# sandialabs/implicit-sph

Measured on AMD Instinct MI355X. Metric: pressure-Poisson solves/sec (3D TGV, 1M particles per GPU, GMRES(50)+block-Jacobi ILU(0), tol 1e-8), higher is better.
Workload: dtype f64; 1 GPU; 3D Taylor-Green vortex, 100^3 particles per GPU, Wendland cut=2h (BASELINE configs[1]), state after one Lagrangian step (mode=advect); rows_per_gpu=1000000, global_rows=1000000, nnz_per_gpu=103845090, solver=FGMRES(50) DGKS tol 1e-8, right prec, precond=bjacobi-ilu0, atom_order=lexicographic, library_row_order=bricks, parallelism=domain bricks 1x1x1, RCCL halo + all-reduce, restarts=1, converged=1

## Files before the change

implicit-sph_amd/csrc/block_helmholtz.hpp:

```cpp
#pragma once
#include "assemble.hpp"

namespace isph {

inline bool sell_cols16(isph_ctx *ctx, const Sell &S);


struct BlockHelmholtzArgs {
  HelmholtzArgs h;
  double beta;
  const double *normal;
  int *bcol[9];
  double *bval[9];
};

__global__ __launch_bounds__(kBlock) void k_asm_block_helmholtz(AsmTables T, BlockHelmholtzArgs A,
                                                                const long long *__restrict__ slice_off,
                                                                double *__restrict__ b) {
  const HelmholtzArgs &a = A.h;
  const int i = xcd_block() * blockDim.x + threadIdx.x;
  const int lane = threadIdx.x & 63;
  const int dim = T.dim, d2 = dim * dim;
  if (i >= a.nlocal) {
    const int nslices = (a.nlocal + kSlice - 1) / kSlice;
// ... 335 lines not shown
        }
        if (rc == ISPH_SUCCESS) rc = (T.sorted && n > 32768) ? sell_set_wmax(ctx, B) : sell_sort_rows(ctx, B);
      }
      if (rc == ISPH_SUCCESS && T.sorted && n > 32768 && sell_cols16(ctx, A0->S)) {
        const Sell &S0 = A0->S;
        for (int q = 1; q < d2 && rc == ISPH_SUCCESS; ++q) {
          if (!blk[q]) continue;
          Sell &B = blk[q]->S;
          rc = B.col16.reserve((size_t)S0.stored);
          if (rc == ISPH_SUCCESS) rc = B.wtab.reserve((size_t)S0.nslices * 64);
          if (rc == ISPH_SUCCESS &&
              (hipMemcpyAsync(B.col16.p, S0.col16.p, sizeof(unsigned short) * (size_t)S0.stored, hipMemcpyDeviceToDevice, ctx->stream) != hipSuccess ||
               hipMemcpyAsync(B.wtab.p, S0.wtab.p, sizeof(int) * (size_t)S0.nslices * 64, hipMemcpyDeviceToDevice, ctx->stream) != hipSuccess))
            rc = fail("copy failed", __FILE__, __LINE__);
          if (rc == ISPH_SUCCESS) B.c16_state = 1;
        }
      }
      if (rc == ISPH_SUCCESS && !on_device &&
          hipMemcpyAsync(b_out, db, sizeof(double) * (size_t)lda * dim, hipMemcpyDeviceToHost, ctx->stream) != hipSuccess)
        rc = fail("copy failed", __FILE__, __LINE__);
      if (hipStreamSynchronize(ctx->stream) != hipSuccess || hipGetLastError() != hipSuccess)
        rc = fail("block assembly kernel failed", __FILE__, __LINE__);
    }
    if (rc == ISPH_SUCCESS) {
      long long tot = 0;
      rc = sell_sum_rowlen(ctx, A0->S, &tot);
      for (int q = 0; q < d2; ++q)
        if (blk[q]) blk[q]->S.nnz = tot;
    }
  }
// ... 14 lines not shown
```

implicit-sph_amd/csrc/core.hpp:

```cpp
#pragma once
#include "common.hpp"
#include "order.hpp"
#include "sell.hpp"

namespace isph { struct HostStager; }

struct isph_neigh_layout {
  const void *nptr = nullptr;
  const int *nidx = nullptr, *colmap = nullptr;
  const void *order = nullptr;
  int n = -1, is_sorted = 0;
  isph::DevBuf<long long> off;
  isph::DevBuf<int> idx, len, sorted;
  void release() { off.release(); idx.release(); len.release(); sorted.release(); nptr = nullptr; nidx = colmap = nullptr; order = nullptr; n = -1; is_sorted = 0; }
};

struct isph_neigh_map {
  const int *rowsrc = nullptr, *idmap = nullptr, *colmap_key = nullptr;
  const int *colkey = nullptr;
  const void *order = nullptr;
};

struct isph_table_cache {
  int ntypes = -1, kernel = -1, dim = -1;
// ... 29 lines not shown
  size_t ev_used = 0;
  std::vector<hipEvent_t> hev;
  size_t hev_used = 0;
  hipEvent_t ev0 = nullptr, ev1 = nullptr;
  hipEvent_t ev_fetch = nullptr;
  std::vector<hipEvent_t> ev_ls;
  hipStream_t comm_stream = nullptr;
  hipEvent_t ev_pack = nullptr, ev_halo = nullptr;
  isph::DevBuf<double> xghost;
  isph::HostStager *stager = nullptr;
  bool neigh_hold = false;
  bool pattern_hold = false;
  isph_neigh_layout neigh_cache[2];
  isph_table_cache tables;
  int ordering = 1;
  isph::OrderBox box;
  isph_neigh_map nmap;
  isph::RowOrderPtr held_order;
  const void *held_key[2] = {nullptr, nullptr};
};

namespace isph {
enum ProfClass { PROF_SPMV = 0, PROF_PREC_APPLY, PROF_MULTI_DOT, PROF_MULTI_AXPY_DOT, PROF_MULTI_AXPY_NORM, PROF_ILU_EXTRACT,
                 PROF_ILU_SCHEDULE, PROF_ILU_FACTOR, PROF_NCLASS };
struct ProfScope {
  isph_ctx *c;
  size_t slot = (size_t)-1;
  ProfScope(isph_ctx *ctx, int cls, hipStream_t st = nullptr) : c(ctx) {
    if (!c || !c->profile || (st && st != c->stream)) return;
    if (c->ev_used + 2 > c->ev.size()) {
// ... 60 lines not shown
```

implicit-sph_amd/csrc/ingress.hpp:

```cpp
#pragma once
#include <atomic>
#include <chrono>
#include <cstdint>
#include <condition_variable>
#include <functional>
#include <thread>
#if defined(__x86_64__)
#include <immintrin.h>
#endif

#include "core.hpp"
#include "ilu.hpp"
#include "pattern.hpp"

namespace isph {

#if defined(__x86_64__)
__attribute__((target("avx2"))) inline void stage_copy_avx2(void *dst, const void *src, size_t bytes) {
  char *d = static_cast<char *>(dst);
  const char *s = static_cast<const char *>(src);
  size_t k = 0;
  while (k < bytes && (reinterpret_cast<uintptr_t>(d + k) & 31)) { d[k] = s[k]; ++k; }
  for (; k + 128 <= bytes; k += 128) {
    const __m256i a = _mm256_loadu_si256(reinterpret_cast<const __m256i *>(s + k));
// ... 434 lines not shown
  H->stats[2] = since();
  if (!copies_ok ||
      hipMemcpyAsync(flags, H->flag.p, 2 * sizeof(int), hipMemcpyDeviceToHost, ctx->stream) != hipSuccess ||
      hipStreamSynchronize(ctx->stream) != hipSuccess || hip_err.load())
    if (rc == ISPH_SUCCESS) rc = fail("CSR->SELL conversion failed", __FILE__, __LINE__);
  H->stats[3] = since();
  ISPH_CHECK(rc);
  ISPH_REQUIRE(!bad_col.load(), "column index out of range");
  if (flags[0]) {
    ISPH_CHECK(sell_sort_rows(ctx, S));
    ISPH_CHECK_HIP(hipStreamSynchronize(ctx->stream));
  }
  if (was_unsorted) *was_unsorted = flags[0] != 0;
  if (S.col16.p != nullptr) {
    S.c16_state = flags[1] ? -1 : flags[0] ? 0 : 1;
    if (S.c16_state != 1) { S.col16.release(); S.wtab.release(); }
  }
  ISPH_CHECK_HIP(hipGetLastError());
  if (ctx->pattern_hold && pattern_mappable(S)) {
    DevTmp<int> debase;
    if (gat) {
      std::vector<int> eb((size_t)nrow);
      for (int r = 0; r < nrow; ++r) eb[(size_t)r] = gat->src_rowptr[gat->perm[r]];
      ISPH_CHECK(debase.reserve((size_t)nrow));
      ISPH_CHECK_HIP(hipMemcpyAsync(debase.p, eb.data(), sizeof(int) * (size_t)nrow, hipMemcpyHostToDevice, ctx->stream));
      ISPH_CHECK_HIP(hipStreamSynchronize(ctx->stream));
    }
    ISPH_CHECK(pattern_build<int>(ctx, g.A, g.drp.p, nullptr, ck, gat ? gat->colren : nullptr, gat ? gat->nren : 0,
                                  gat ? debase.p : nullptr));
  }
  H->bytes_sent = sent + 4 * ((long long)nrow + 1);
// ... 232 lines not shown
```

implicit-sph_amd/csrc/isph_capi.hip:

```cpp
#include <algorithm>
#include <numeric>

#include "assemble.hpp"
#include "operators.hpp"
#include "block_helmholtz.hpp"
#include "core.hpp"
#include "ilu.hpp"
#include "krylov.hpp"
#include "sell.hpp"
#include "solver.hpp"
#include "chebyshev.hpp"
#include "amg.hpp"
#include "schwarz.hpp"
#include "gcrodr.hpp"
#include "ingress.hpp"

namespace isph {
thread_local std::string g_last_error;

}

struct isph_overlap {
  int n = 0, next = 0, combine = 0;
  isph_schwarz *inner = nullptr;
// ... 930 lines not shown
    ISPH_CHECK_HIP(hipStreamSynchronize(ctx->stream));
  }
  return ISPH_SUCCESS;
}

int isph_mat_info(const isph_mat *A, long long info[6]) {
  ISPH_REQUIRE(A && info, "NULL argument");
  info[0] = A->S.nrow; info[1] = A->S.ncol; info[2] = A->S.nnz; info[3] = A->S.nslices;
  info[4] = A->S.stored; info[5] = A->S.stored * 12 + ((long long)A->S.nslices + 1) * 8;
  return ISPH_SUCCESS;
}

int isph_mat_column_bits(isph_ctx *ctx, const isph_mat *A, int *bits) {
  ISPH_REQUIRE(ctx && A && bits, "NULL argument");
  *bits = (!A->local && !A->aux && sell_cols16(ctx, A->S)) ? 16 : 32;
  return ISPH_SUCCESS;
}

int isph_mat_export_rows(isph_ctx *ctx, const isph_mat *A, int row_begin, int nrows, long long *rowptr, int *colidx,
                         double *val, long long capacity) {
  ISPH_REQUIRE(ctx && A && rowptr && colidx && val, "NULL argument");
  const Sell &S = A->S;
  ISPH_REQUIRE(row_begin >= 0 && nrows >= 0 && (long long)row_begin + nrows <= S.nrow, "row range outside the matrix");
  if (A->order && nrows > 0) {
    std::vector<int> hperm((size_t)S.nrow), hiperm((size_t)S.nrow);
    ISPH_CHECK_HIP(hipMemcpyAsync(hperm.data(), A->order->perm.p, sizeof(int) * hperm.size(), hipMemcpyDeviceToHost, ctx->stream));
    ISPH_CHECK_HIP(hipMemcpyAsync(hiperm.data(), A->order->iperm.p, sizeof(int) * hiperm.size(), hipMemcpyDeviceToHost, ctx->stream));
    ISPH_CHECK_HIP(hipStreamSynchronize(ctx->stream));
    isph_mat plain;
    plain.S = S;
// ... 142 lines not shown
    return ISPH_SUCCESS;
  }
  ISPH_CHECK(ctx->xdev.reserve((size_t)S.ncol));
  ISPH_CHECK(ctx->bdev.reserve((size_t)(S.nrow > 0 ? S.nrow : 1)));
  ISPH_CHECK_HIP(hipMemcpyAsync(ctx->xdev.p, x, sizeof(double) * nx, hipMemcpyHostToDevice, ctx->stream));
  if (S.ncol > S.nrow && A->halo.npeers == 0) {
    int nbp = 0;
    const int grid = spmv_grid(S.nslices, &nbp);
    hipLaunchKernelGGL((k_sell_spmv<8, false, true>), dim3(grid), dim3(kBlock), 0, ctx->stream, S.nrow, S.nslices, nbp,
                       S.slice_off.p, S.col.p, S.val.p, (const double *)ctx->xdev.p, ctx->bdev.p, (const double *)nullptr,
                       (double *)nullptr);
  } else {
    ISPH_CHECK(spmv_dev(ctx, A, ctx->xdev.p, ctx->bdev.p, nullptr));
  }
  ISPH_CHECK_HIP(hipMemcpyAsync(y, ctx->bdev.p, sizeof(double) * (size_t)S.nrow, hipMemcpyDeviceToHost, ctx->stream));
  ISPH_CHECK_HIP(hipStreamSynchronize(ctx->stream));
  ISPH_CHECK_HIP(hipGetLastError());
  return ISPH_SUCCESS;
}

int isph_spmv_time(isph_ctx *ctx, const isph_mat *A, const double *x_dev, double *y_dev, int reps, int variant, double *avg_ms) {
  ISPH_REQUIRE(ctx && A && x_dev && y_dev && avg_ms && reps > 0, "bad argument");
  const Sell &S = A->S;
  ISPH_REQUIRE(S.ncol == S.nrow || A->halo.npeers > 0, "ghost columns without halo plan");
  if (S.ncol != S.nrow) {
    ISPH_CHECK_HIP(hipEventRecord(ctx->ev0, ctx->stream));
    for (int r = 0; r < reps; ++r) ISPH_CHECK(spmv_dev(ctx, A, x_dev, y_dev, nullptr));
    ISPH_CHECK_HIP(hipEventRecord(ctx->ev1, ctx->stream));
    ISPH_CHECK_HIP(hipEventSynchronize(ctx->ev1));
    float msh = 0.f;
// ... 988 lines not shown
```

implicit-sph_amd/csrc/sell.hpp:

```cpp
#pragma once
#include "common.hpp"

namespace isph {

struct Sell {
  int nrow = 0, ncol = 0, nslices = 0, wmax = 0;
  long long nnz = 0, stored = 0;
  DevBuf<long long> slice_off;
  DevBuf<int> rowlen;
  DevBuf<int> col;
  DevBuf<double> val;
  mutable DevBuf<unsigned short> col16;
  mutable DevBuf<int> wtab;
  mutable int c16_state = 0;
  void release() { slice_off.release(); rowlen.release(); col.release(); val.release(); col16.release(); wtab.release(); c16_state = 0; }
};

__device__ __forceinline__ unsigned amg_like_hash(int x) {
  unsigned h = (unsigned)x;
  h ^= h >> 16; h *= 0x7feb352dU; h ^= h >> 15; h *= 0x846ca68bU; h ^= h >> 16;
  return h;
}

__device__ __forceinline__ long long sell_pos(long long off, int lane, int k) {
  return off + (long long)(k >> 1) * 128 + lane * 2 + (k & 1);
}

template <class OFF>
__global__ void k_csr_rowlen_slicew(int nrow, const OFF *__restrict__ rowptr, int *__restrict__ rowlen,
                                    long long *__restrict__ slice_cnt) {
// ... 496 lines not shown
    const unsigned lo = cc & 0xffffu, hi = cc >> 16;
    acc0 = fma((double)vv.x, x_at<GHOST>(x, xg, nrow, tw[lo >> 10] | (int)(lo & 1023u)), acc0);
    acc1 = fma((double)vv.y, x_at<GHOST>(x, xg, nrow, tw[hi >> 10] | (int)(hi & 1023u)), acc1);
  }
  const int row = slice * kSlice + lane;
  double r = acc0 + acc1;
  if (alpha != 1.0) r *= alpha;
  if (badd != nullptr && row < nrow) r += (double)badd[row];
  if (row < nrow) y[row] = (YT)r;
  if (DOT) {
    const double d = wave_sum(row < nrow ? r * nvec[row] : 0.0);
    if (lane == 0) dot_partial[slice] = d;
  }
}

struct SpmmVecs {
  const double *x[4];
  double *y[4];
};
template <int NV>
__global__ __launch_bounds__(kBlock) void k_sell_spmm16(int nrow, int nslices, int nblocks_padded,
                                                        const long long *__restrict__ slice_off,
                                                        const unsigned short *__restrict__ c16,
                                                        const int *__restrict__ wtab, const double *__restrict__ sval,
                                                        SpmmVecs V) {
  constexpr int UNROLL = 4;
  __shared__ int tab[kBlock / kWave][64];
  const int b = xcd_remap(blockIdx.x, nblocks_padded);
  const int wave = threadIdx.x >> 6;
  const int slice = b * (kBlock / kWave) + wave;
// ... 91 lines not shown
```

implicit-sph_amd/csrc/solver.hpp:

```cpp
#pragma once
#include <cmath>
#include <type_traits>

#include "comm.hpp"
#include "core.hpp"
#include "gmres_host.hpp"
#include "krylov.hpp"

namespace isph {

int prec_apply_dev(isph_ctx *ctx, const isph_prec *M, const double *r, double *z);
int prec_apply_multi_dev(isph_ctx *ctx, const isph_prec *M, int K, const double *const *rs, double *const *zs);

inline int allreduce_inplace(isph_ctx *ctx, double *d, int count) {
  return comm_allreduce(ctx, d, count,  0, ctx->stream);
}

enum { SC_DOT = 0 , SC_Y = 64 , SC_MISC = 128, SC_COUNT = 160 };

constexpr int kMaxLockstep = 4;

inline int ensure_scalars(isph_ctx *ctx) {
  ISPH_CHECK(ctx->dscal.reserve(SC_COUNT * kMaxLockstep));
  ISPH_CHECK(ctx->partial.reserve((size_t)kMaxRedBlocks * 66));
// ... 55 lines not shown
  if (flag.reserve(1) != ISPH_SUCCESS || S.col16.reserve((size_t)S.stored) != ISPH_SUCCESS ||
      S.wtab.reserve((size_t)S.nslices * 64) != ISPH_SUCCESS) { flag.release(); return false; }
  int h = 0;
  if (hipMemsetAsync(flag.p, 0, sizeof(int), ctx->stream) == hipSuccess) {
    hipLaunchKernelGGL(k_sell_compress_cols, dim3((S.nslices + 3) / 4), dim3(kBlock), 0, ctx->stream, 0, S.nslices,
                       (const long long *)S.slice_off.p, (const int *)S.col.p, S.col16.p, S.wtab.p, flag.p);
    if (hipMemcpyAsync(&h, flag.p, sizeof(int), hipMemcpyDeviceToHost, ctx->stream) == hipSuccess &&
        hipStreamSynchronize(ctx->stream) == hipSuccess && hipGetLastError() == hipSuccess && h == 0)
      S.c16_state = 1;
  }
  flag.release();
  if (S.c16_state < 0) { S.col16.release(); S.wtab.release(); }
  return S.c16_state > 0;
}

template <bool DOT, bool LIST, bool GHOST>
inline void spmv_launch(isph_ctx *ctx, const Sell &S, bool c16, int nsl, const int *list, const double *x, const double *xg,
                        double *y, const double *nvec, const double *badd = nullptr, double alpha = 1.0,
                        const float *val32 = nullptr) {
  if (nsl <= 0) return;
  int nbp = 0;
  const int grid = spmv_grid(nsl, &nbp);
  double *part = DOT ? ctx->partial.p : nullptr;
  if (val32 && c16)
    hipLaunchKernelGGL((k_sell_spmv16<8, false, LIST, GHOST, float>), dim3(grid), dim3(kBlock), 0, ctx->stream, S.nrow, nsl, nbp,
                       S.slice_off.p, S.col16.p, S.wtab.p, val32, x, y, nvec, part, list, xg, badd, alpha);
  else if (val32)
    hipLaunchKernelGGL((k_sell_spmv<8, false, true, LIST, GHOST, float>), dim3(grid), dim3(kBlock), 0, ctx->stream, S.nrow, nsl, nbp,
                       S.slice_off.p, S.col.p, val32, x, y, nvec, part, list, xg, badd, alpha);
  else if (c16)
    hipLaunchKernelGGL((k_sell_spmv16<8, DOT, LIST, GHOST>), dim3(grid), dim3(kBlock), 0, ctx->stream, S.nrow, nsl, nbp,
                       S.slice_off.p, S.col16.p, S.wtab.p, S.val.p, x, y, nvec, part, list, xg, badd, alpha);
  else
    hipLaunchKernelGGL((k_sell_spmv<8, DOT, true, LIST, GHOST>), dim3(grid), dim3(kBlock), 0, ctx->stream, S.nrow, nsl, nbp,
                       S.slice_off.p, S.col.p, S.val.p, x, y, nvec, part, list, xg, badd, alpha);
}

inline int spmv_dev(isph_ctx *ctx, const isph_mat *A, const double *x, double *y, const double *nvec, const double *badd = nullptr,
                    double alpha = 1.0, const float *val32 = nullptr) {
  const Sell &S = A->S;
  const bool halo = !A->local && (S.ncol != S.nrow || A->halo.nsend > 0);
  const bool c16 = !A->local && !A->aux && sell_cols16(ctx, S);
  ISPH_REQUIRE(nvec == nullptr || (badd == nullptr && alpha == 1.0 && val32 == nullptr), "spmv: the dot epilogue takes the plain product");
  ProfScope prof((A->local || A->aux) ? nullptr : ctx, PROF_SPMV);
  if (nvec)
    ISPH_CHECK(ctx->partial.reserve((size_t)S.nslices > (size_t)kMaxRedBlocks * 66 ? (size_t)S.nslices : (size_t)kMaxRedBlocks * 66));
  if (!halo) {
    if (nvec) spmv_launch<true, false, false>(ctx, S, c16, S.nslices, nullptr, x, nullptr, y, nvec);
    else spmv_launch<false, false, false>(ctx, S, c16, S.nslices, nullptr, x, nullptr, y, nvec, badd, alpha, val32);
  } else {
    const isph_halo &H = A->halo;
    hipEvent_t *hev = nullptr;
    if (ctx->profile && !A->aux && !A->local) {
      if (ctx->hev_used + 3 > ctx->hev.size())
        for (int k = 0; k < 3; ++k) { hipEvent_t e = nullptr; ISPH_CHECK_HIP(hipEventCreate(&e)); ctx->hev.push_back(e); }
      hev = ctx->hev.data() + ctx->hev_used;
      ctx->hev_used += 3;
    }
    ISPH_CHECK(halo_begin(ctx, A, x, hev));
    if (nvec) spmv_launch<true, true, false>(ctx, S, c16, H.n_int, H.list_int.p, x, nullptr, y, nvec);
    else spmv_launch<false, true, false>(ctx, S, c16, H.n_int, H.list_int.p, x, nullptr, y, nvec, badd, alpha, val32);
    if (hev) ISPH_CHECK_HIP(hipEventRecord(hev[2], ctx->stream));
    ISPH_CHECK_HIP(hipStreamWaitEvent(ctx->stream, ctx->ev_halo, 0));
    if (nvec) spmv_launch<true, true, true>(ctx, S, c16, H.n_bnd, H.list_bnd.p, x, ctx->xghost.p, y, nvec);
// ... 595 lines not shown
```

implicit-sph_amd/hip.py:

```python
import ctypes as C
import sys
import os

import numpy as np

from . import build as _build

UID_BYTES = 128
NOT_SINGULAR, NULLSPACE, PINZERO, DOUBLEDIAG = 0, 1, 2, 3
KERNELS = {"wendland": 0, "quintic": 1, "cubic": 2}

EXPORTS = [
    "isph_ctx_create", "isph_comm_unique_id", "isph_ctx_create_dist", "isph_ctx_create_hostcomm", "isph_ctx_sync", "isph_ctx_destroy", "isph_pool_trim", "isph_pool_set_cap", "isph_set_exact_stream_threshold", "isph_pool_cached_bytes", "isph_pool_info", "isph_halo_create", "isph_halo_forward", "isph_halo_destroy", "isph_prec_create_overlap",
    "isph_last_error", "isph_mat_create_csr", "isph_mat_create_csr_bjacobi", "isph_mat_create_csr_blocks", "isph_mat_create_csr_coords", "isph_mat_create_csr_coords_bjacobi", "isph_ingress_info", "isph_mat_set_halo", "isph_mat_info", "isph_mat_export_csr", "isph_mat_export_rows", "isph_mat_column_bits",
    "isph_mat_destroy", "isph_spmv", "isph_spmv_time", "isph_prec_create", "isph_prec_create_blocks", "isph_prec_create_blocks_fill", "isph_prec_apply",
    "isph_prec_export_ilu", "isph_prec_nnz", "isph_prec_info", "isph_prec_destroy", "isph_solver_params_default", "isph_solve",
    "isph_ctx_set_profile", "isph_ctx_hold_neighbours", "isph_ctx_profile_read", "isph_ctx_set_ordering", "isph_ctx_set_periodic_box", "isph_mat_ordering_info", "isph_mat_ordering", "isph_mat_ordering_faces", "isph_ctx_halo_profile_read", "isph_ctx_comm_info", "isph_device_identity", "isph_assemble_poisson", "isph_assemble_helmholtz", "isph_assemble_solute_transport", "isph_assemble_applied_potential", "isph_compute_volumes", "isph_compute_pnd", "isph_compute_corrections", "isph_gradient", "isph_divergence", "isph_correct_velocity_pressure",
    "isph_advance_begin", "isph_advance_end", "isph_compute_shift", "isph_apply_shift", "isph_shift_particles",
    "isph_solve_block", "isph_assemble_block_helmholtz", "isph_amg_params_default", "isph_prec_create_amg", "isph_prec_amg_levels", "isph_prec_amg_info",
    "isph_prec_amg_export", "isph_prec_amg_aggregates", "isph_prec_amg_path",
    "isph_schwarz_params_default", "isph_prec_create_schwarz", "isph_prec_schwarz_info", "isph_prec_schwarz_timing", "isph_prec_schwarz_export",
    "isph_pb_params_default", "isph_assemble_poisson_boltzmann", "isph_pb_residual", "isph_pb_jacobian", "isph_solve_poisson_boltzmann",
    "isph_compute_normals", "isph_csf_params_default", "isph_csf_phase_normal", "isph_csf_force", "isph_surface_tension_csf", "isph_pairwise_force",
    "isph_smooth_field", "isph_ek_params_default", "isph_electrostatic_force", "isph_random_stress_tensor", "isph_random_stress_force",
    "isph_force_from_random_stress", "isph_cheb_params_default", "isph_prec_create_chebyshev", "isph_prec_value_bits", "isph_prec_cycle_bits",
    "isph_prec_eig_estimate",
    "isph_ilu_params_default", "isph_prec_create_ilu",
    "isph_nlist_build", "isph_nlist_info", "isph_nlist_get", "isph_nlist_destroy",
    "isph_ctx_hold_pattern", "isph_mat_update_values", "isph_mat_pattern_info", "isph_prec_refactor",
# ... 125 lines not shown
                                          C.c_int, C.c_void_p]
        L.isph_mat_create_csr_bjacobi.argtypes = [C.c_void_p, C.c_int, C.c_int, C.c_void_p, C.c_void_p, C.c_void_p,
                                                  C.c_int, C.c_void_p, C.c_void_p]
        L.isph_mat_create_csr_blocks.argtypes = [C.c_void_p, C.c_int, C.c_int, C.c_void_p, C.c_void_p, C.c_void_p,
                                                 C.c_int, C.c_void_p, C.c_void_p, C.c_void_p]
        L.isph_mat_create_csr_coords.argtypes = [C.c_void_p, C.c_int, C.c_int, C.c_void_p, C.c_void_p, C.c_void_p, C.c_int,
                                                 C.c_void_p, C.c_void_p, C.c_void_p, C.c_void_p]
        L.isph_mat_create_csr_coords_bjacobi.argtypes = [C.c_void_p, C.c_int, C.c_int, C.c_void_p, C.c_void_p, C.c_void_p, C.c_int,
                                                         C.c_void_p, C.c_void_p, C.c_void_p, C.c_void_p, C.c_void_p]
        L.isph_mat_set_halo.argtypes = [C.c_void_p, C.c_void_p, C.c_int, C.c_void_p, C.c_void_p, C.c_void_p,
                                        C.c_void_p]
        L.isph_mat_info.argtypes = [C.c_void_p, C.c_void_p]
        L.isph_mat_export_csr.argtypes = [C.c_void_p, C.c_void_p, C.c_void_p, C.c_void_p, C.c_void_p]
        L.isph_mat_export_rows.argtypes = [C.c_void_p, C.c_void_p, C.c_int, C.c_int, C.c_void_p, C.c_void_p, C.c_void_p, C.c_longlong]
        L.isph_mat_column_bits.argtypes = [C.c_void_p, C.c_void_p, C.c_void_p]
        L.isph_mat_destroy.argtypes = [C.c_void_p]
        L.isph_spmv.argtypes = [C.c_void_p, C.c_void_p, C.c_void_p, C.c_void_p, C.c_int]
        L.isph_spmv_time.argtypes = [C.c_void_p, C.c_void_p, C.c_void_p, C.c_void_p, C.c_int, C.c_int, C.c_void_p]
        L.isph_prec_create.argtypes = [C.c_void_p, C.c_void_p, C.c_char_p, C.c_int, C.c_void_p]
        L.isph_prec_create_blocks.argtypes = [C.c_void_p, C.c_void_p, C.c_int, C.c_void_p, C.c_void_p]
        L.isph_prec_create_blocks_fill.argtypes = [C.c_void_p, C.c_void_p, C.c_int, C.c_void_p, C.c_int, C.c_void_p]
        L.isph_prec_apply.argtypes = [C.c_void_p, C.c_void_p, C.c_void_p, C.c_void_p, C.c_int]
        L.isph_prec_export_ilu.argtypes = [C.c_void_p, C.c_void_p, C.c_void_p, C.c_void_p, C.c_void_p]
        L.isph_prec_destroy.argtypes = [C.c_void_p]
        L.isph_prec_info.argtypes = [C.c_void_p, C.c_void_p, C.c_void_p]
        L.isph_solve.argtypes = [C.c_void_p, C.c_void_p, C.c_void_p, C.c_void_p, C.c_void_p, C.c_int, C.c_int,
                                 C.c_int, C.c_void_p, C.c_void_p, C.c_void_p, C.c_int]
        L.isph_assemble_poisson.argtypes = [C.c_void_p, C.c_void_p, C.c_int, C.c_double, C.c_void_p, C.c_void_p,
                                            C.c_int, C.c_int, C.c_int, C.c_void_p, C.c_void_p, C.c_int]
        L.isph_compute_volumes.argtypes = [C.c_void_p, C.c_void_p, C.c_void_p, C.c_int]
# ... 190 lines not shown
        if transport is not None:
            _check(lib().isph_ctx_create_hostcomm(device, sp, rank, nranks, C.byref(transport), C.byref(self.h)))
        elif nranks > 1 or uid is not None:
            _check(lib().isph_ctx_create_dist(device, sp, rank, nranks, uid, C.byref(self.h)))
        else:
            _check(lib().isph_ctx_create(device, sp, C.byref(self.h)))
        ordering = DEFAULT_ORDERING if ordering is None else ordering
        self.ordering = "bricks" if ordering is None else ordering
        if ordering is not None:
            self.set_ordering(ordering)

    def set_ordering(self, mode):
        _check(lib().isph_ctx_set_ordering(self.h, ORDERINGS[mode]))
        self.ordering = mode

    def set_periodic_box(self, lo=None, hi=None, periodic=None):
        if lo is None:
            _check(lib().isph_ctx_set_periodic_box(self.h, None, None, None))
            return
        a = (C.c_double * 3)(*[float(v) for v in (list(lo) + [0.0] * 3)[:3]])
        b = (C.c_double * 3)(*[float(v) for v in (list(hi) + [0.0] * 3)[:3]])
        p = (C.c_int * 3)(*[int(v) for v in (list(periodic) + [0] * 3)[:3]])
        _check(lib().isph_ctx_set_periodic_box(self.h, a, b, p))

    @staticmethod
    def unique_id():
        buf = C.create_string_buffer(UID_BYTES)
        _check(lib().isph_comm_unique_id(buf))
        return buf.raw

# ... 170 lines not shown
        _check(lib().isph_mat_export_csr(self.ctx.h, self.h, _ptr(rp), _ptr(ci), _ptr(v)))
        return rp, ci, v

    def export_rows(self, row_begin, nrows, capacity=None):
        cap = int(capacity if capacity is not None else nrows * 4096)
        rp = np.zeros(nrows + 1, dtype=np.int64)
        ci = np.zeros(cap, dtype=np.int32)
        v = np.zeros(cap)
        _check(lib().isph_mat_export_rows(self.ctx.h, self.h, int(row_begin), int(nrows), _ptr(rp), _ptr(ci), _ptr(v), cap))
        return rp, ci[:rp[-1]], v[:rp[-1]]

    def column_bits(self):
        b = C.c_int()
        _check(lib().isph_mat_column_bits(self.ctx.h, self.h, C.byref(b)))
        return b.value

    def update_values(self, val):
        val = _f64(val)
        _need(val, self.info()["nnz"], "val [nnz]")
        _check(lib().isph_mat_update_values(self.ctx.h, self.h, _ptr(val), _on_device(val)))

    def pattern_info(self):
        a = (C.c_longlong * 3)()
        _check(lib().isph_mat_pattern_info(self.h, a))
        return int(a[0]), int(a[1]), int(a[2])

    def sampled_product(self, x, nsamples=64, rows_per_sample=64, seed=0):
        n = self.info()["nrow"]
        xh = x.detach().cpu().numpy() if _is_torch(x) else np.asarray(x)
        rng = np.random.default_rng(seed)
# ... 903 lines not shown
```

include/isph_hip.h:

```cpp
#ifndef ISPH_HIP_H
#define ISPH_HIP_H

#ifdef __cplusplus
extern "C" {
#endif

typedef struct isph_ctx isph_ctx;
typedef struct isph_mat isph_mat;
typedef struct isph_prec isph_prec;

#define ISPH_SUCCESS 0
#define ISPH_FAILURE (-1)
#define ISPH_UID_BYTES 128


int isph_ctx_create(int device, void *stream, isph_ctx **ctx);
int isph_comm_unique_id(char *uid);
int isph_ctx_create_dist(int device, void *stream, int rank, int nranks,
                         const char *uid, isph_ctx **ctx);
typedef struct {
  void *user;
  int (*exchange)(void *user, int npeers, const int *peer, const double *send, const long long *send_off,
                  double *recv, const long long *recv_off);
  int (*allreduce)(void *user, double *buf, int count, int op);
// ... 32 lines not shown
int isph_mat_update_values(isph_ctx *ctx, isph_mat *A, const double *val , int on_device);
int isph_mat_pattern_info(const isph_mat *A, long long info[3]);
int isph_mat_set_halo(isph_ctx *ctx, isph_mat *A, int npeers, const int *peer_rank,
                      const int *send_ptr, const int *send_idx, const int *recv_ptr);
typedef struct isph_halo_plan isph_halo_plan;
int isph_halo_create(isph_ctx *ctx, int nlocal, int npeers, const int *peer_rank, const int *send_ptr,
                     const int *send_idx, const int *recv_ptr, isph_halo_plan **plan);
int isph_halo_forward(isph_ctx *ctx, const isph_halo_plan *plan, const double *x , double *ghosts ,
                      int ncomp, int on_device);
void isph_halo_destroy(isph_halo_plan *plan);
int isph_mat_info(const isph_mat *A, long long info[6]);
int isph_mat_export_csr(isph_ctx *ctx, const isph_mat *A, int *rowptr, int *colidx, double *val);
int isph_mat_export_rows(isph_ctx *ctx, const isph_mat *A, int row_begin, int nrows, long long *rowptr, int *colidx,
                         double *val, long long capacity);
int isph_mat_column_bits(isph_ctx *ctx, const isph_mat *A, int *bits);
void isph_mat_destroy(isph_mat *A);

int isph_spmv(isph_ctx *ctx, const isph_mat *A, const double *x ,
              double *y , int on_device);
int isph_spmv_time(isph_ctx *ctx, const isph_mat *A, const double *x_dev, double *y_dev,
                   int reps, int variant, double *avg_ms);


int isph_prec_create(isph_ctx *ctx, const isph_mat *A, const char *type, int block_size,
                     isph_prec **M);
int isph_prec_create_blocks(isph_ctx *ctx, const isph_mat *A, int nblocks, const int *block_ptr, isph_prec **M);
int isph_prec_create_blocks_fill(isph_ctx *ctx, const isph_mat *A, int nblocks, const int *block_ptr, int level_of_fill,
                                 isph_prec **M);
typedef struct {
  int level_of_fill;
  int block_size;
  int nblocks;
  const int *block_ptr;
  int value_bits;
// ... 274 lines not shown
```

Baseline: 25.54 solves/s (1M-particle bricks; x n_gpus under weak scaling).

## Add 8-bit per-slice delta-dictionary column codes for SELL SpMV

Result: no change. 25.70 solves/s (1M-particle bricks; x n_gpus under weak scaling), median of 5 (+0.7%).

```diff
diff --git a/implicit-sph_amd/csrc/block_helmholtz.hpp b/implicit-sph_amd/csrc/block_helmholtz.hpp
--- a/implicit-sph_amd/csrc/block_helmholtz.hpp
+++ b/implicit-sph_amd/csrc/block_helmholtz.hpp
@@ -373,6 +373,15 @@
                hipMemcpyAsync(B.wtab.p, S0.wtab.p, sizeof(int) * (size_t)S0.nslices * 64, hipMemcpyDeviceToDevice, ctx->stream) != hipSuccess))
             rc = fail("copy failed", __FILE__, __LINE__);
           if (rc == ISPH_SUCCESS) B.c16_state = 1;
+          if (rc == ISPH_SUCCESS && S0.c8_state == 1) {
+            rc = B.code8.reserve((size_t)S0.code8_bytes());
+            if (rc == ISPH_SUCCESS) rc = B.dtab.reserve((size_t)S0.nslices * 256);
+            if (rc == ISPH_SUCCESS &&
+                (hipMemcpyAsync(B.code8.p, S0.code8.p, (size_t)S0.code8_bytes(), hipMemcpyDeviceToDevice, ctx->stream) != hipSuccess ||
+                 hipMemcpyAsync(B.dtab.p, S0.dtab.p, sizeof(int) * (size_t)S0.nslices * 256, hipMemcpyDeviceToDevice, ctx->stream) != hipSuccess))
+              rc = fail("copy failed", __FILE__, __LINE__);
+            if (rc == ISPH_SUCCESS) B.c8_state = 1;
+          }
         }
       }
       if (rc == ISPH_SUCCESS && !on_device &&
diff --git a/implicit-sph_amd/csrc/core.hpp b/implicit-sph_amd/csrc/core.hpp
--- a/implicit-sph_amd/csrc/core.hpp
+++ b/implicit-sph_amd/csrc/core.hpp
@@ -67,6 +67,7 @@
   isph_neigh_layout neigh_cache[2];
   isph_table_cache tables;
   int ordering = 1;
+  int column_form = 0;
   isph::OrderBox box;
   isph_neigh_map nmap;
   isph::RowOrderPtr held_order;
diff --git a/implicit-sph_amd/csrc/ingress.hpp b/implicit-sph_amd/csrc/ingress.hpp
--- a/implicit-sph_amd/csrc/ingress.hpp
+++ b/implicit-sph_amd/csrc/ingress.hpp
@@ -472,7 +472,7 @@
   if (was_unsorted) *was_unsorted = flags[0] != 0;
   if (S.col16.p != nullptr) {
     S.c16_state = flags[1] ? -1 : flags[0] ? 0 : 1;
-    if (S.c16_state != 1) { S.col16.release(); S.wtab.release(); }
+    if (S.c16_state != 1) { S.col16.release(); S.wtab.release(); S.release_cols8(); }
   }
   ISPH_CHECK_HIP(hipGetLastError());
   if (ctx->pattern_hold && pattern_mappable(S)) {
diff --git a/implicit-sph_amd/csrc/isph_capi.hip b/implicit-sph_amd/csrc/isph_capi.hip
--- a/implicit-sph_amd/csrc/isph_capi.hip
+++ b/implicit-sph_amd/csrc/isph_capi.hip
@@ -968,6 +968,32 @@
 int isph_mat_column_bits(isph_ctx *ctx, const isph_mat *A, int *bits) {
   ISPH_REQUIRE(ctx && A && bits, "NULL argument");
   *bits = (!A->local && !A->aux && sell_cols16(ctx, A->S)) ? 16 : 32;
+  return ISPH_SUCCESS;
+}
+
+int isph_ctx_set_column_form(isph_ctx *ctx, int form) {
+  ISPH_REQUIRE(ctx && (form == 0 || form == 16 || form == 8), "bad column form (0, 16 or 8)");
+  ctx->column_form = form;
+  return ISPH_SUCCESS;
+}
+
+int isph_mat_column_codes8(isph_ctx *ctx, const isph_mat *A, int *used) {
+  ISPH_REQUIRE(ctx && A && used, "NULL argument");
+  const Sell &S = A->S;
+  const bool halo = !A->local && (S.ncol != S.nrow || A->halo.nsend > 0);
+  *used = (!A->local && !A->aux && !halo && spmv_wants_cols8(ctx) && sell_cols16(ctx, S) && sell_cols8(ctx, S)) ? 1 : 0;
+  return ISPH_SUCCESS;
+}
+
+int isph_mat_export_cols8(isph_ctx *ctx, const isph_mat *A, long long sizes[2], int *dtab, unsigned char *codes) {
+  ISPH_REQUIRE(ctx && A && sizes, "NULL argument");
+  const Sell &S = A->S;
+  ISPH_REQUIRE(S.c8_state == 1, "the matrix has no 8-bit column codes (isph_mat_column_codes8 builds them where it can)");
+  sizes[0] = (long long)S.nslices * 256;
+  sizes[1] = S.code8_bytes();
+  if (dtab) ISPH_CHECK_HIP(hipMemcpyAsync(dtab, S.dtab.p, sizeof(int) * (size_t)sizes[0], hipMemcpyDeviceToHost, ctx->stream));
+  if (codes) ISPH_CHECK_HIP(hipMemcpyAsync(codes, S.code8.p, (size_t)sizes[1], hipMemcpyDeviceToHost, ctx->stream));
+  ISPH_CHECK_HIP(hipStreamSynchronize(ctx->stream));
   return ISPH_SUCCESS;
 }
 
@@ -1140,6 +1166,42 @@
     ISPH_CHECK(spmv_dev(ctx, A, ctx->xdev.p, ctx->bdev.p, nullptr));
   }
   ISPH_CHECK_HIP(hipMemcpyAsync(y, ctx->bdev.p, sizeof(double) * (size_t)S.nrow, hipMemcpyDeviceToHost, ctx->stream));
+  ISPH_CHECK_HIP(hipStreamSynchronize(ctx->stream));
+  ISPH_CHECK_HIP(hipGetLastError());
+  return ISPH_SUCCESS;
+}
+
+int isph_spmv_dot(isph_ctx *ctx, const isph_mat *A, const double *x, const double *nvec, double *y, double *dot) {
+  ISPH_REQUIRE(ctx && A && x && nvec && y && dot, "NULL argument");
+  const Sell &S = A->S;
+  ISPH_REQUIRE(S.ncol == S.nrow || A->halo.npeers > 0, "ghost columns without halo plan");
+  const size_t n = (size_t)S.nrow;
+  DevTmp<double> xc, nc, xi, ni, yi;
+  ISPH_CHECK(xc.reserve(n + 64));
+  ISPH_CHECK(nc.reserve(n + 64));
+  ISPH_CHECK(yi.reserve(n + 64));
+  ISPH_CHECK_HIP(hipMemcpyAsync(xc.p, x, sizeof(double) * n, hipMemcpyHostToDevice, ctx->stream));
+  ISPH_CHECK_HIP(hipMemcpyAsync(nc.p, nvec, sizeof(double) * n, hipMemcpyHostToDevice, ctx->stream));
+  const double *dx = xc.p, *dn = nc.p;
+  if (A->order && n > 0) {
+    ISPH_CHECK(xi.reserve(n + 64));
+    ISPH_CHECK(ni.reserve(n + 64));
+    hipLaunchKernelGGL((k_perm_gather<double>), dim3(perm_grid((long long)n)), dim3(kBlock), 0, ctx->stream, (long long)n, S.nrow, 1,
+                       (const int *)A->order->perm.p, (const double *)xc.p, xi.p);
+    hipLaunchKernelGGL((k_perm_gather<double>), dim3(perm_grid((long long)n)), dim3(kBlock), 0, ctx->stream, (long long)n, S.nrow, 1,
+                       (const int *)A->order->perm.p, (const double *)nc.p, ni.p);
+    dx = xi.p;
+    dn = ni.p;
+  }
+  ISPH_CHECK(spmv_dev(ctx, A, dx, yi.p, dn));
+  const double *dy = yi.p;
+  if (A->order && n > 0) {
+    hipLaunchKernelGGL((k_perm_scatter<double>), dim3(perm_grid(S.nrow)), dim3(kBlock), 0, ctx->stream, S.nrow,
+                       (const int *)A->order->perm.p, (const double *)yi.p, xc.p);
+    dy = xc.p;
+  }
+  ISPH_CHECK_HIP(hipMemcpyAsync(y, dy, sizeof(double) * n, hipMemcpyDeviceToHost, ctx->stream));
+  ISPH_CHECK_HIP(hipMemcpyAsync(dot, ctx->dscal.p + SC_MISC, sizeof(double), hipMemcpyDeviceToHost, ctx->stream));
   ISPH_CHECK_HIP(hipStreamSynchronize(ctx->stream));
   ISPH_CHECK_HIP(hipGetLastError());
   return ISPH_SUCCESS;
diff --git a/implicit-sph_amd/csrc/sell.hpp b/implicit-sph_amd/csrc/sell.hpp
--- a/implicit-sph_amd/csrc/sell.hpp
+++ b/implicit-sph_amd/csrc/sell.hpp
@@ -13,7 +13,15 @@
   mutable DevBuf<unsigned short> col16;
   mutable DevBuf<int> wtab;
   mutable int c16_state = 0;
-  void release() { slice_off.release(); rowlen.release(); col.release(); val.release(); col16.release(); wtab.release(); c16_state = 0; }
+  mutable DevBuf<unsigned char> code8;
+  mutable DevBuf<int> dtab;
+  mutable int c8_state = 0;
+  long long code8_bytes() const { return ((stored >> 10) + nslices) * 1024; }
+  void release_cols8() const { code8.release(); dtab.release(); c8_state = 0; }
+  void release() {
+    slice_off.release(); rowlen.release(); col.release(); val.release(); col16.release(); wtab.release(); c16_state = 0;
+    release_cols8();
+  }
 };
 
 __device__ __forceinline__ unsigned amg_like_hash(int x) {
@@ -540,6 +548,162 @@
   }
 }
 
+constexpr int kDeltaEmpty = (int)0x80000000;
+constexpr bool kCols8Default = true;
+
+__global__ __launch_bounds__(kBlock) void k_sell_encode_cols8(int nslices, const long long *__restrict__ slice_off,
+                                                              const int *__restrict__ scol, unsigned char *__restrict__ code8,
+                                                              int *__restrict__ dtab, int *__restrict__ fail) {
+  __shared__ int tab[kBlock / kWave][256];
+  const int wave = threadIdx.x >> 6, lane = threadIdx.x & 63;
+  const int slice = blockIdx.x * (kBlock / kWave) + wave;
+  if (slice >= nslices) return;
+#pragma unroll
+  for (int i = 0; i < 4; ++i) tab[wave][lane + 64 * i] = kDeltaEmpty;
+  __builtin_amdgcn_fence(__ATOMIC_RELEASE, "wavefront");
+  __builtin_amdgcn_wave_barrier();
+  const long long off = slice_off[slice];
+  const int npair = (int)((slice_off[slice + 1] - off) >> 7);
+  const int2 *__restrict__ c = reinterpret_cast<const int2 *>(scol + off) + lane;
+  bool bad = false;
+  int prev = slice * kSlice, last = kDeltaEmpty;
+  for (int q = 0; q < npair; ++q) {
+    const int2 cc = c[q * 64];
+    const int d[2] = {cc.x - prev, cc.y - cc.x};
+    prev = cc.y;
+#pragma unroll
+    for (int h = 0; h < 2; ++h) {
+      if (d[h] == last) continue;
+      last = d[h];
+      int slot = (int)(amg_like_hash(d[h]) & 255u);
+      for (int tries = 0; tries < 256; ++tries) {
+        int old = __atomic_load_n(&tab[wave][slot], __ATOMIC_RELAXED);
+        if (old == kDeltaEmpty) old = atomicCAS(&tab[wave][slot], kDeltaEmpty, d[h]);
+        if (old == kDeltaEmpty || old == d[h]) break;
+        slot = (slot + 1) & 255;
+        if (tries == 255) bad = true;
+      }
+    }
+  }
+  __builtin_amdgcn_fence(__ATOMIC_RELEASE, "wavefront");
+  __builtin_amdgcn_wave_barrier();
+  if (__ballot(bad)) { if (lane == 0) atomicOr(fail, 1); return; }
+#pragma unroll
+  for (int i = 0; i < 4; ++i) {
+    const int t = tab[wave][lane + 64 * i];
+    dtab[(long long)slice * 256 + lane + 64 * i] = t == kDeltaEmpty ? 0 : t;
+  }
+  uint4 *__restrict__ out = reinterpret_cast<uint4 *>(code8 + ((off >> 10) + slice) * 1024) + lane;
+  prev = slice * kSlice;
+  last = kDeltaEmpty;
+  unsigned last_slot = 0;
+  const int ngroup = npair / 8 + 1;
+  for (int g = 0; g < ngroup; ++g) {
+    unsigned w[4] = {0u, 0u, 0u, 0u};
+#pragma unroll
+    for (int j = 0; j < 8; ++j) {
+      const int q = 8 * g + j;
+      if (q >= npair) break;
+      const int2 cc = c[q * 64];
+      const int d[2] = {cc.x - prev, cc.y - cc.x};
+      prev = cc.y;
+#pragma unroll
+      for (int h = 0; h < 2; ++h) {
+        if (d[h] != last) {
+          unsigned slot = amg_like_hash(d[h]) & 255u;
+          while (tab[wave][slot] != d[h]) slot = (slot + 1) & 255u;
+          last = d[h];
+          last_slot = slot;
+        }
+        w[j >> 1] |= last_slot << (16 * (j & 1) + 8 * h);
+      }
+    }
+    out[g * 64] = make_uint4(w[0], w[1], w[2], w[3]);
+  }
+}
+
+typedef unsigned u32x4 __attribute__((ext_vector_type(4)));
+template <int UNROLL, bool DOT>
+__global__ __launch_bounds__(kBlock) void k_sell_spmv8(int nrow, int nslices, int nblocks_padded,
+                                                       const long long *__restrict__ slice_off,
+                                                       const unsigned char *__restrict__ code8,
+                                                       const int *__restrict__ dtab, const double *__restrict__ sval,
+                                                       const double *__restrict__ x, double *__restrict__ y,
+                                                       const double *__restrict__ nvec, double *__restrict__ dot_partial,
+                                                       const double *badd = nullptr, double alpha = 1.0) {
+  static_assert(UNROLL == 8, "a 16-byte group of codes carries 8 pairs");
+  __shared__ __attribute__((aligned(16))) int tab[kBlock / kWave][256];
+  const int b = xcd_remap(blockIdx.x, nblocks_padded);
+  const int wave = threadIdx.x >> 6;
+  const int slice = __builtin_amdgcn_readfirstlane(b * (kBlock / kWave) + wave);
+  if (slice >= nslices) return;
+  const int lane = threadIdx.x & 63;
+  const long long off = slice_off[slice];
+  const int npair = (int)((slice_off[slice + 1] - off) >> 7);
+  const double2 *__restrict__ v = reinterpret_cast<const double2 *>(sval + off) + lane;
+  const u32x4 *__restrict__ cg = reinterpret_cast<const u32x4 *>(code8 + ((off >> 10) + slice) * 1024) + lane;
+  const int4 t4 = reinterpret_cast<const int4 *>(dtab + (long long)slice * 256)[lane];
+  u32x4 cw = __builtin_nontemporal_load(cg);
+  reinterpret_cast<int4 *>(tab[wave])[lane] = t4;
+  __builtin_amdgcn_fence(__ATOMIC_RELEASE, "wavefront");
+  __builtin_amdgcn_wave_barrier();
+  const int *__restrict__ tw = tab[wave];
+  int col = slice * kSlice;
+  double acc0 = 0.0, acc1 = 0.0;
+  int q = 0;
+  for (; q + UNROLL <= npair; q += UNROLL) {
+    double2 vv[UNROLL];
+#pragma unroll
+    for (int u = 0; u < UNROLL; ++u) {
+      vv[u].x = __builtin_nontemporal_load(&v[(q + u) * 64].x);
+      vv[u].y = __builtin_nontemporal_load(&v[(q + u) * 64].y);
+    }
+    const u32x4 cn = __builtin_nontemporal_load(cg + ((q >> 3) + 1) * 64);
+    int ca[UNROLL], cb[UNROLL];
+#pragma unroll
+    for (int u = 0; u < UNROLL; ++u) {
+      const unsigned h = cw[u >> 1] >> (16 * (u & 1));
+      col += tw[h & 255u];
+      ca[u] = col;
+      col += tw[(h >> 8) & 255u];
+      cb[u] = col;
+    }
+    double xa[UNROLL], xb[UNROLL];
+#pragma unroll
+    for (int u = 0; u < UNROLL; ++u) {
+      xa[u] = x[ca[u]];
+      xb[u] = x[cb[u]];
+    }
+#pragma unroll
+    for (int u = 0; u < UNROLL; ++u) {
+      acc0 = fma(vv[u].x, xa[u], acc0);
+      acc1 = fma(vv[u].y, xb[u], acc1);
+    }
+    cw = cn;
+  }
+  for (; q < npair; ++q) {
+    const double2 vv = v[q * 64];
+    col += tw[cw[0] & 255u];
+    const int ca = col;
+    col += tw[(cw[0] >> 8) & 255u];
+    acc0 = fma(vv.x, x[ca], acc0);
+    acc1 = fma(vv.y, x[col], acc1);
+    cw[0] = (cw[0] >> 16) | (cw[1] << 16);
+    cw[1] = (cw[1] >> 16) | (cw[2] << 16);
+    cw[2] = (cw[2] >> 16) | (cw[3] << 16);
+    cw[3] >>= 16;
+  }
+  const int row = slice * kSlice + lane;
+  double r = acc0 + acc1;
+  if (alpha != 1.0) r *= alpha;
+  if (badd != nullptr && row < nrow) r += (double)badd[row];
+  if (row < nrow) y[row] = r;
+  if (DOT) {
+    const double d = wave_sum(row < nrow ? r * nvec[row] : 0.0);
+    if (lane == 0) dot_partial[slice] = d;
+  }
+}
+
 struct SpmmVecs {
   const double *x[4];
   double *y[4];
diff --git a/implicit-sph_amd/csrc/solver.hpp b/implicit-sph_amd/csrc/solver.hpp
--- a/implicit-sph_amd/csrc/solver.hpp
+++ b/implicit-sph_amd/csrc/solver.hpp
@@ -93,15 +93,41 @@
   return S.c16_state > 0;
 }
 
+inline bool sell_cols8(isph_ctx *ctx, const Sell &S) {
+  if (S.c8_state != 0) return S.c8_state > 0;
+  S.c8_state = -1;
+  if (S.c16_state <= 0 || S.nslices == 0 || S.stored == 0) return false;
+  DevTmp<int> flag;
+  if (flag.reserve(1) != ISPH_SUCCESS || S.code8.reserve((size_t)S.code8_bytes()) != ISPH_SUCCESS ||
+      S.dtab.reserve((size_t)S.nslices * 256) != ISPH_SUCCESS) { flag.release(); S.code8.release(); S.dtab.release(); return false; }
+  int h = 0;
+  if (hipMemsetAsync(flag.p, 0, sizeof(int), ctx->stream) == hipSuccess &&
+      hipMemsetAsync(S.code8.p, 0, (size_t)S.code8_bytes(), ctx->stream) == hipSuccess) {
+    hipLaunchKernelGGL(k_sell_encode_cols8, dim3((S.nslices + 3) / 4), dim3(kBlock), 0, ctx->stream, S.nslices,
+                       (const long long *)S.slice_off.p, (const int *)S.col.p, S.code8.p, S.dtab.p, flag.p);
+    if (hipMemcpyAsync(&h, flag.p, sizeof(int), hipMemcpyDeviceToHost, ctx->stream) == hipSuccess &&
+        hipStreamSynchronize(ctx->stream) == hipSuccess && hipGetLastError() == hipSuccess && h == 0)
+      S.c8_state = 1;
+  }
+  flag.release();
+  if (S.c8_state < 0) { S.code8.release(); S.dtab.release(); }
+  return S.c8_state > 0;
+}
+
+inline bool spmv_wants_cols8(const isph_ctx *ctx) { return ctx->column_form == 8 || (ctx->column_form == 0 && kCols8Default); }
+
 template <bool DOT, bool LIST, bool GHOST>
 inline void spmv_launch(isph_ctx *ctx, const Sell &S, bool c16, int nsl, const int *list, const double *x, const double *xg,
                         double *y, const double *nvec, const double *badd = nullptr, double alpha = 1.0,
-                        const float *val32 = nullptr) {
+                        const float *val32 = nullptr, bool c8 = false) {
   if (nsl <= 0) return;
   int nbp = 0;
   const int grid = spmv_grid(nsl, &nbp);
   double *part = DOT ? ctx->partial.p : nullptr;
-  if (val32 && c16)
+  if (c8 && !LIST && !GHOST && !val32)
+    hipLaunchKernelGGL((k_sell_spmv8<8, DOT>), dim3(grid), dim3(kBlock), 0, ctx->stream, S.nrow, nsl, nbp,
+                       S.slice_off.p, S.code8.p, S.dtab.p, S.val.p, x, y, nvec, part, badd, alpha);
+  else if (val32 && c16)
     hipLaunchKernelGGL((k_sell_spmv16<8, false, LIST, GHOST, float>), dim3(grid), dim3(kBlock), 0, ctx->stream, S.nrow, nsl, nbp,
                        S.slice_off.p, S.col16.p, S.wtab.p, val32, x, y, nvec, part, list, xg, badd, alpha);
   else if (val32)
@@ -120,13 +146,14 @@
   const Sell &S = A->S;
   const bool halo = !A->local && (S.ncol != S.nrow || A->halo.nsend > 0);
   const bool c16 = !A->local && !A->aux && sell_cols16(ctx, S);
+  const bool c8 = c16 && !halo && val32 == nullptr && spmv_wants_cols8(ctx) && sell_cols8(ctx, S);
   ISPH_REQUIRE(nvec == nullptr || (badd == nullptr && alpha == 1.0 && val32 == nullptr), "spmv: the dot epilogue takes the plain product");
   ProfScope prof((A->local || A->aux) ? nullptr : ctx, PROF_SPMV);
   if (nvec)
     ISPH_CHECK(ctx->partial.reserve((size_t)S.nslices > (size_t)kMaxRedBlocks * 66 ? (size_t)S.nslices : (size_t)kMaxRedBlocks * 66));
   if (!halo) {
-    if (nvec) spmv_launch<true, false, false>(ctx, S, c16, S.nslices, nullptr, x, nullptr, y, nvec);
-    else spmv_launch<false, false, false>(ctx, S, c16, S.nslices, nullptr, x, nullptr, y, nvec, badd, alpha, val32);
+    if (nvec) spmv_launch<true, false, false>(ctx, S, c16, S.nslices, nullptr, x, nullptr, y, nvec, nullptr, 1.0, nullptr, c8);
+    else spmv_launch<false, false, false>(ctx, S, c16, S.nslices, nullptr, x, nullptr, y, nvec, badd, alpha, val32, c8);
   } else {
     const isph_halo &H = A->halo;
     hipEvent_t *hev = nullptr;
diff --git a/implicit-sph_amd/hip.py b/implicit-sph_amd/hip.py
--- a/implicit-sph_amd/hip.py
+++ b/implicit-sph_amd/hip.py
@@ -13,6 +13,7 @@
 EXPORTS = [
     "isph_ctx_create", "isph_comm_unique_id", "isph_ctx_create_dist", "isph_ctx_create_hostcomm", "isph_ctx_sync", "isph_ctx_destroy", "isph_pool_trim", "isph_pool_set_cap", "isph_set_exact_stream_threshold", "isph_pool_cached_bytes", "isph_pool_info", "isph_halo_create", "isph_halo_forward", "isph_halo_destroy", "isph_prec_create_overlap",
     "isph_last_error", "isph_mat_create_csr", "isph_mat_create_csr_bjacobi", "isph_mat_create_csr_blocks", "isph_mat_create_csr_coords", "isph_mat_create_csr_coords_bjacobi", "isph_ingress_info", "isph_mat_set_halo", "isph_mat_info", "isph_mat_export_csr", "isph_mat_export_rows", "isph_mat_column_bits",
+    "isph_ctx_set_column_form", "isph_mat_column_codes8", "isph_mat_export_cols8", "isph_spmv_dot",
     "isph_mat_destroy", "isph_spmv", "isph_spmv_time", "isph_prec_create", "isph_prec_create_blocks", "isph_prec_create_blocks_fill", "isph_prec_apply",
     "isph_prec_export_ilu", "isph_prec_nnz", "isph_prec_info", "isph_prec_destroy", "isph_solver_params_default", "isph_solve",
     "isph_ctx_set_profile", "isph_ctx_hold_neighbours", "isph_ctx_profile_read", "isph_ctx_set_ordering", "isph_ctx_set_periodic_box", "isph_mat_ordering_info", "isph_mat_ordering", "isph_mat_ordering_faces", "isph_ctx_halo_profile_read", "isph_ctx_comm_info", "isph_device_identity", "isph_assemble_poisson", "isph_assemble_helmholtz", "isph_assemble_solute_transport", "isph_assemble_applied_potential", "isph_compute_volumes", "isph_compute_pnd", "isph_compute_corrections", "isph_gradient", "isph_divergence", "isph_correct_velocity_pressure",
@@ -168,6 +169,10 @@
         L.isph_mat_export_csr.argtypes = [C.c_void_p, C.c_void_p, C.c_void_p, C.c_void_p, C.c_void_p]
         L.isph_mat_export_rows.argtypes = [C.c_void_p, C.c_void_p, C.c_int, C.c_int, C.c_void_p, C.c_void_p, C.c_void_p, C.c_longlong]
         L.isph_mat_column_bits.argtypes = [C.c_void_p, C.c_void_p, C.c_void_p]
+        L.isph_ctx_set_column_form.argtypes = [C.c_void_p, C.c_int]
+        L.isph_mat_column_codes8.argtypes = [C.c_void_p, C.c_void_p, C.c_void_p]
+        L.isph_mat_export_cols8.argtypes = [C.c_void_p, C.c_void_p, C.c_void_p, C.c_void_p, C.c_void_p]
+        L.isph_spmv_dot.argtypes = [C.c_void_p, C.c_void_p, C.c_void_p, C.c_void_p, C.c_void_p, C.c_void_p]
         L.isph_mat_destroy.argtypes = [C.c_void_p]
         L.isph_spmv.argtypes = [C.c_void_p, C.c_void_p, C.c_void_p, C.c_void_p, C.c_int]
         L.isph_spmv_time.argtypes = [C.c_void_p, C.c_void_p, C.c_void_p, C.c_void_p, C.c_int, C.c_int, C.c_void_p]
@@ -388,6 +393,9 @@
         _check(lib().isph_ctx_set_ordering(self.h, ORDERINGS[mode]))
         self.ordering = mode
 
+    def set_column_form(self, form):
+        _check(lib().isph_ctx_set_column_form(self.h, int(form)))
+
     def set_periodic_box(self, lo=None, hi=None, periodic=None):
         if lo is None:
             _check(lib().isph_ctx_set_periodic_box(self.h, None, None, None))
@@ -588,6 +596,28 @@
         b = C.c_int()
         _check(lib().isph_mat_column_bits(self.ctx.h, self.h, C.byref(b)))
         return b.value
+
+    def column_codes8(self):
+        u = C.c_int()
+        _check(lib().isph_mat_column_codes8(self.ctx.h, self.h, C.byref(u)))
+        return bool(u.value)
+
+    def export_cols8(self):
+        sz = (C.c_longlong * 2)()
+        _check(lib().isph_mat_export_cols8(self.ctx.h, self.h, sz, None, None))
+        dtab = np.zeros(int(sz[0]), dtype=np.int32)
+        codes = np.zeros(int(sz[1]), dtype=np.uint8)
+        _check(lib().isph_mat_export_cols8(self.ctx.h, self.h, sz, _ptr(dtab), _ptr(codes)))
+        return dtab.reshape(-1, 256), codes
+
+    def spmv_dot(self, x, nvec):
+        n = self.info()["nrow"]
+        x, nvec = np.ascontiguousarray(x, dtype=np.float64), np.ascontiguousarray(nvec, dtype=np.float64)
+        _need(x, n, "x [nrow]")
+        _need(nvec, n, "nvec [nrow]")
+        y, d = np.zeros(n), C.c_double()
+        _check(lib().isph_spmv_dot(self.ctx.h, self.h, _ptr(x), _ptr(nvec), _ptr(y), C.byref(d)))
+        return y, d.value
 
     def update_values(self, val):
         val = _f64(val)
diff --git a/include/isph_hip.h b/include/isph_hip.h
--- a/include/isph_hip.h
+++ b/include/isph_hip.h
@@ -70,10 +70,15 @@
 int isph_mat_export_rows(isph_ctx *ctx, const isph_mat *A, int row_begin, int nrows, long long *rowptr, int *colidx,
                          double *val, long long capacity);
 int isph_mat_column_bits(isph_ctx *ctx, const isph_mat *A, int *bits);
+int isph_ctx_set_column_form(isph_ctx *ctx, int form);
+int isph_mat_column_codes8(isph_ctx *ctx, const isph_mat *A, int *used);
+int isph_mat_export_cols8(isph_ctx *ctx, const isph_mat *A, long long sizes[2], int *dtab, unsigned char *codes);
 void isph_mat_destroy(isph_mat *A);
 
 int isph_spmv(isph_ctx *ctx, const isph_mat *A, const double *x ,
               double *y , int on_device);
+int isph_spmv_dot(isph_ctx *ctx, const isph_mat *A, const double *x , const double *nvec , double *y ,
+                  double *dot);
 int isph_spmv_time(isph_ctx *ctx, const isph_mat *A, const double *x_dev, double *y_dev,
                    int reps, int variant, double *avg_ms);
 
```
